# stephane-caron/qpmpc

Hardware: AMD Instinct MI355X
Metric: MPC QP builds+solves/sec (batched) (higher is better)
Workload: dtype f64

## Files before the change

qpmpc_amd/csrc/mpcqp_quad.hip:

```cpp
#include <hip/hip_runtime.h>
#include <math.h>
#include <stdint.h>
#include <type_traits>

#include "mpcqp.h"
#include "mpcqp_internal.h"
#include "mpcqp_quad_common.h"

namespace mpcqp {

namespace quad {

constexpr int MMAX = 32;
constexpr int MK = 2;

}

using namespace quad;

template <int NX, bool ORD, int WPB, bool SLIM, bool MODEL = false, bool GEN = false>
__global__ void __launch_bounds__(64 * WPB, SLIM ? 2 : 1)
    mpcqp_quad_kernel(const double *__restrict__ gA, const double *__restrict__ gB, const double *__restrict__ gC,
                      const double *__restrict__ ge, const double *__restrict__ gx0, const double *__restrict__ ggoal,
                      const double *__restrict__ gtgt, double *__restrict__ oU, double *__restrict__ olam, int32_t *__restrict__ ostatus,
                      int32_t *__restrict__ oiters, const KernelArgs ka, const int64_t batch)
{
    using T = double;
    extern __shared__ __attribute__((aligned(16))) unsigned char smem_raw[];
    {
        const int64_t b0 = ka.A.batch_stride, b1 = ka.B.batch_stride, b2 = ka.C.batch_stride, b3 = ka.e.batch_stride,
                      b4 = ka.x0.batch_stride, b5 = ka.goal.batch_stride;
        const int64_t s0 = ka.A.step_stride, s1 = ka.B.step_stride, s2 = ka.C.step_stride, s3 = ka.e.step_stride;
        asm volatile("" ::"s"(b0), "s"(b1), "s"(b2), "s"(b3), "s"(b4), "s"(b5), "s"(s0), "s"(s1), "s"(s2), "s"(s3), "s"(ka.N), "s"(ka.nu),
                     "s"(ka.flags), "s"(ka.probe), "s"(gA), "s"(gB), "s"(gC), "s"(ge), "s"(gx0), "s"(ggoal), "s"(ka.n), "s"(ka.m),
                     "s"(batch));
    }
    const int lane = threadIdx.x & 63;
    const int wv = threadIdx.x >> 6;
    const int rb = lane & 48;
    const int l = lane & 15;
    int64_t prob = 4 * ((int64_t)blockIdx.x * WPB + wv) + (rb >> 4);
    const bool valid = prob < batch;
    prob = valid ? prob : batch - 1;
    if constexpr (ORD) {
        const int64_t o = ka.order[prob];
        prob = o < 0 ? 0 : (o >= batch ? batch - 1 : o);
    }
    using CV = Carve<SLIM>;
    constexpr int LDM = CV::LDM, PER = CV::PER;
    T *sm = (T *)smem_raw + (4 * wv + (rb >> 4)) * PER;
    const int n = ka.n, m = ka.m;
    const int row0 = l, row1 = l + NV;
    const bool isc0 = row0 < m, isc1 = row1 < m;
    const T INF = HUGE_VAL;
    constexpr int GS = 33;
    T *Gimg = sm + CV::OFF_M, *Ml = sm + CV::OFF_M;
    T *LTp = sm + CV::OFF_LT + (l * (31 - l)) / 2 - (l + 1);
    T *LTimg = sm + CV::OFF_LT, *Timg = sm + CV::OFF_T, *kAv = sm + CV::OFF_KA;
    int *actv = reinterpret_cast<int *>(sm + CV::OFF_ACT);

    long long *stamp = ka.probe ? (long long *)ka.probe + prob * 16 : nullptr;
    auto tick = [&](int slot) {
        if (stamp && l == 0 && valid) {
            stamp[slot] = (long long)__builtin_readcyclecounter();
            if (slot == 0 || slot == 6) stamp[slot ? 13 : 12] = (long long)__builtin_amdgcn_s_memrealtime();
        }
    };
    tick(0);

    T hval0, hval1;
    bool notpd = false;
    T RM0[NV], RM1[NV], RLt[NV];
    T wv_ = T(0);
    if constexpr (MODEL) {
        const T *model = gA;
        const ModelLayout ml = make_model_layout(ka.nx, ka.N, n, m);
        const int nxr = ka.nx, nT = ka.N * ka.nx;
        const T *x0 = gx0 + prob * ka.x0.batch_stride;
        const T *goal = ggoal ? ggoal + prob * ka.goal.batch_stride : nullptr;
        const T *tgt = gtgt ? gtgt + prob * ka.targets.batch_stride : nullptr;
        notpd = model[ml.total] != T(0);
        {
            T r0[NV], r1[NV];
            ld16(r0, model + ml.off_M + (size_t)(isc0 ? row0 : 0) * NV);
            ld16(r1, model + ml.off_M + (size_t)(isc1 ? row1 : 0) * NV);
            ld16(RLt, model + ml.off_LinvT + (size_t)l * NV);
#pragma unroll
            for (int k = 0; k < NV; ++k) {
                RM0[k] = isc0 ? r0[k] : T(0);
                RM1[k] = isc1 ? r1[k] : T(0);
            }
        }
        auto bound = [&](int row, bool isc) {
            if (!isc) return INF;
            const int mkr = ka.mk, kq = mkr == 2 ? row >> 1 : row / mkr;
            T hh = ge ? ge[prob * ka.e.batch_stride + kq * ka.e.step_stride + (row - kq * mkr)] : model[ml.off_e + row];
            for (int c = 0; c < nxr; ++c) hh -= model[ml.off_Hx + (size_t)row * nxr + c] * x0[c];
            return hh;
        };
        hval0 = bound(row0, isc0);
        hval1 = bound(row1, isc1);
        for (int c = 0; c < nxr; ++c) wv_ += model[ml.off_Wx + (size_t)l * nxr + c] * x0[c];
        if ((ka.flags & MPCQP_Q_TERMINAL) && goal)
            for (int c = 0; c < nxr; ++c) wv_ -= model[ml.off_Wg + (size_t)l * nxr + c] * goal[c];
        if ((ka.flags & MPCQP_Q_STAGE) && tgt)
            for (int j2 = 0; j2 < nT; ++j2) wv_ -= model[ml.off_Wt + (size_t)l * nT + j2] * tgt[j2];
        tick(1);
    } else {
    T Pr[NV];
    T qa;
    T g15a = T(0), g15b = T(0);
    {
        constexpr bool WIDE = GEN && NX > 6;
        const int nx = WIDE ? ka.nx : NX;
        const int nu = ka.nu, N = ka.N;
        constexpr int MKG = GEN ? 4 : MK;
        const int mk = GEN ? ka.mk : MK;
        auto stepof = [&](int row) { return mk == 2 ? row >> 1 : (mk == 1 ? row : (mk == 4 ? row >> 2 : row / 3)); };
        const T *A = gA + prob * ka.A.batch_stride;
        const T *B = gB + prob * ka.B.batch_stride;
        const bool hasC = !GEN || gC != nullptr;
        const T *Cm = hasC ? gC + prob * ka.C.batch_stride : A;
        const T *x0 = gx0 + prob * ka.x0.batch_stride;
        const T *goal = ggoal ? ggoal + prob * ka.goal.batch_stride : nullptr;
        const int sA = ka.A.step_stride ? nx * nx : 0, sB = ka.B.step_stride ? nx * nu : 0, sC = (hasC && ka.C.step_stride) ? mk * nx : 0;
        const bool termP = ka.flags & MPCQP_P_TERMINAL, termQ = (ka.flags & MPCQP_Q_TERMINAL) && goal;
        const T *Dm = (GEN && ka.D.ptr) ? (const T *)ka.D.ptr + prob * ka.D.batch_stride : nullptr;
        const T *tgt = (GEN && gtgt) ? gtgt + prob * ka.targets.batch_stride : nullptr;
        const int sD = (GEN && ka.D.step_stride) ? mk * nu : 0;
        const bool stageP = GEN && (ka.flags & MPCQP_P_STAGE), stageQ = GEN && (ka.flags & MPCQP_Q_STAGE) && tgt;
        constexpr int NAe = NX * NX, NEe = NAe + MKG * NX;
        const int NEr = hasC ? NAe + mk * NX : NAe;
        const bool col = (l < n);
        const int j = col ? (nu == 1 ? l : l / nu) : -1, ii = col ? l - j * nu : 0;
        const int64_t eb = prob * ka.e.batch_stride;
        const int kq0 = stepof(row0), kq1 = stepof(row1);
        const T eval0 = isc0 ? ge[eb + kq0 * ka.e.step_stride + (row0 - kq0 * mk)] : INF;
        const T eval1 = isc1 ? ge[eb + kq1 * ka.e.step_stride + (row1 - kq1 * mk)] : INF;
        const bool xl15 = (l == NV - 1);
        T v[NX], gref[NX], bcol[NX];
#pragma unroll
        for (int s = 0; s < NX; ++s) {
            v[s] = (xl15 && s < nx) ? x0[s < nx ? s : 0] : T(0);
            gref[s] = (termQ && s < nx) ? goal[s < nx ? s : 0] : T(0);
        }
#pragma unroll
        for (int r = 0; r < NX; ++r) bcol[r] = (col && r < nx) ? B[j * sB + (r < nx ? r : 0) * nu + ii] : T(0);
        T dcol[MKG], d15a = T(0), d15b = T(0), tg[NX];
#pragma unroll
        for (int u = 0; u < NX; ++u) tg[u] = T(0);
#pragma unroll
        for (int i2 = 0; i2 < MKG; ++i2) dcol[i2] = T(0);
        if constexpr (GEN) {
            if (Dm) {
#pragma unroll
                for (int i2 = 0; i2 < MKG; ++i2) dcol[i2] = (col && !xl15 && i2 < mk) ? Dm[j * sD + i2 * nu + ii] : T(0);
                if (n == NV) {
                    const int j15 = nu == 1 ? NV - 1 : (NV - 1) / nu, i15 = NV - 1 - j15 * nu;
                    d15a = (isc0 && kq0 == j15) ? Dm[j15 * sD + (row0 - kq0 * mk) * nu + i15] : T(0);
                    d15b = (isc1 && kq1 == j15) ? Dm[j15 * sD + (row1 - kq1 * mk) * nu + i15] : T(0);
                }
            }
            if (stageQ && !WIDE) {
#pragma unroll
                for (int u = 0; u < NX; ++u) tg[u] = (l + 16 * u < N * NX) ? tgt[l + 16 * u] : T(0);
            }
        }
        if constexpr (!WIDE) {
        constexpr int NOP = (NEe + 15) / 16;
        T op[NOP][NV];
        static_for<0, NOP>([&](auto rc) {
            constexpr int r = decltype(rc)::value;
            const int e = l + 16 * r;
            const bool ok = e < NEr;
            const T *p = (e < NAe) ? A + e : Cm + (ok ? e - NAe : 0);
            const int st = (e < NAe) ? sA : sC;
#pragma unroll
            for (int k = 0; k < NV; ++k) {
                const int kc = (k < N) ? k : N - 1;
                op[r][k] = p[kc * st];
            }
        });
        tick(8);
        const T wu = (T)ka.wu;
        qa = T(0);
#pragma unroll
        for (int b = 0; b < NV; ++b) Pr[b] = (l == b) ? (col ? wu : T(1)) : T(0);
        tick(9);
        auto mac = [&](auto idx, auto kc_, T &acc, T xx) {
            constexpr int IDX = decltype(idx)::value, K = decltype(kc_)::value;
            fmac_bcast<IDX % 16>(acc, op[IDX / 16][K], xx);
        };
        static_for<0, NV>([&](auto kk) {
            constexpr int k = decltype(kk)::value;
            if (k < N) {
                if constexpr (!GEN) {
                    T g[MK];
                    static_for<0, MK>([&](auto i2c) {
                        constexpr int i2 = decltype(i2c)::value;
                        T acc = T(0);
                        static_for<0, NX>([&](auto sc) {
                            constexpr int s2 = decltype(sc)::value;
                            mac(ic<NAe + i2 * NX + s2>{}, kk, acc, v[s2]);
                        });
                        g[i2] = acc;
                    });
#pragma unroll
                    for (int i2 = 0; i2 < MK; ++i2) Gimg[l * GS + k * MK + i2] = g[i2];
                } else {
                    static_for<0, MKG>([&](auto i2c) {
                        constexpr int i2 = decltype(i2c)::value;
                        if (i2 < mk) {
                            T acc = T(0);
                            if (hasC) {
                                static_for<0, NX>([&](auto sc) {
                                    constexpr int s2 = decltype(sc)::value;
                                    mac(ic<NAe + i2 * NX + s2>{}, kk, acc, v[s2]);
                                });
                            }
                            acc += (j == k) ? dcol[i2] : T(0);
                            Gimg[l * GS + k * mk + i2] = acc;
                        }
                    });
                }
                if constexpr (GEN && k >= 1) {
                    if (stageP || stageQ) {
                        const T wxs = (T)ka.wx;
                        static_for<0, NX>([&](auto sc) {
                            constexpr int s2 = decltype(sc)::value;
                            constexpr int te = k * NX + s2;
                            T src = xl15 ? T(0) : v[s2];
                            const T t = wxs * src;
                            if (stageQ) qa += t * (row_bcast<NV - 1>(v[s2]) - row_bcast<te % 16>(tg[te / 16]));
                            if (stageP) {
                                dpp_ready(src);
                                static_for<0, NV>([&](auto bc) { fmac_bcast<decltype(bc)::value>(Pr[decltype(bc)::value], src, t); });
                            }
                        });
                    }
                }
                const T hk = (j == k && !xl15) ? T(1) : T(0);
                T w[NX];
                static_for<0, NX>([&](auto rc) {
                    constexpr int r = decltype(rc)::value;
                    T acc = hk * bcol[r];
                    static_for<0, NX>([&](auto sc) {
                        constexpr int s2 = decltype(sc)::value;
                        mac(ic<r * NX + s2>{}, kk, acc, v[s2]);
                    });
                    w[r] = acc;
                });
#pragma unroll
                for (int r = 0; r < NX; ++r) v[r] = w[r];
            }
        });
        } else {
        tick(8);
        const T wu = (T)ka.wu;
        qa = T(0);
#pragma unroll
        for (int b = 0; b < NV; ++b) Pr[b] = (l == b) ? (col ? wu : T(1)) : T(0);
        tick(9);
        constexpr int NAw = NX * NX, NCw = 4 * NX, NEw = NAw + NCw + NX, NOPW = (NEw + 15) / 16;
        T opw[2][NOPW];
        auto fetch = [&](auto dc, int k) {
            constexpr int d = decltype(dc)::value;
            const int kc = k < N ? k : N - 1;
            static_for<0, NOPW>([&](auto rc) {
                constexpr int r = decltype(rc)::value;
                constexpr int e0 = 16 * r;
                const int e = e0 + l;
                T val;
                if constexpr (e0 < NAw) {
                    const int rr = e / NX, ss = e - rr * NX;
                    const bool ok = rr < nx && ss < nx;
                    val = A[kc * sA + (ok ? rr * nx + ss : 0)];
                    val = ok ? val : T(0);
                } else if constexpr (e0 < NAw + NCw) {
                    const int e2 = e - NAw, i2 = e2 / NX, ss = e2 - i2 * NX;
                    const bool ok = hasC && i2 < mk && ss < nx;
                    val = Cm[ok ? kc * sC + i2 * nx + ss : 0];
                    val = ok ? val : T(0);
                } else {
                    const int ss = e - NAw - NCw;
                    const bool ok = stageQ && ss < nx;
                    val = ok ? tgt[kc * nx + ss] : T(0);
                }
                opw[d][r] = val;
            });
        };
        fetch(ic<0>{}, 0);
        fetch(ic<1>{}, 1);
        const T wxs = (T)ka.wx;
        auto cstep = [&](auto dc, int k) {
            constexpr int d = decltype(dc)::value;
            static_for<0, NOPW>([&](auto rc) { dpp_ready(opw[d][decltype(rc)::value]); });
            static_for<0, 4>([&](auto i2c) {
                constexpr int i2 = decltype(i2c)::value;
                if (i2 < mk) {
                    T acc = T(0);
                    if (hasC) {
                        static_for<0, NX>([&](auto sc) {
                            constexpr int s2 = decltype(sc)::value, E = NAw + i2 * NX + s2;
                            fmac_bcast<E % 16>(acc, opw[d][E / 16], v[s2]);
                        });
                    }
                    acc += (j == k) ? dcol[i2] : T(0);
                    Gimg[l * GS + k * mk + i2] = acc;
                }
            });
            if (k >= 1 && (stageP || stageQ)) {
                static_for<0, NX>([&](auto sc) {
                    constexpr int s2 = decltype(sc)::value, E = NAw + NCw + s2;
                    T src = xl15 ? T(0) : v[s2];
                    const T t = wxs * src;
                    if (stageQ) qa += t * (row_bcast<NV - 1>(v[s2]) - row_bcast<E % 16>(opw[d][E / 16]));
                    if (stageP) {
                        dpp_ready(src);
                        static_for<0, NV>([&](auto bc) { fmac_bcast<decltype(bc)::value>(Pr[decltype(bc)::value], src, t); });
                    }
                });
            }
            const T hk = (j == k && !xl15) ? T(1) : T(0);
            T w[NX];
            static_for<0, NX>([&](auto rc) {
                constexpr int r = decltype(rc)::value;
                T acc = hk * bcol[r];
                static_for<0, NX>([&](auto sc) {
                    constexpr int s2 = decltype(sc)::value, E = r * NX + s2;
                    fmac_bcast<E % 16>(acc, opw[d][E / 16], v[s2]);
                });
                w[r] = acc;
            });
#pragma unroll
            for (int r = 0; r < NX; ++r) v[r] = w[r];
            fetch(dc, k + 2);
        };
        for (int k = 0; k < N; k += 2) {
            cstep(ic<0>{}, k);
            if (k + 1 < N) cstep(ic<1>{}, k + 1);
        }
        }
        tick(10);
        const T wt = (T)ka.wt;
        T x[NX];
#pragma unroll
        for (int s = 0; s < NX; ++s) {
            x[s] = row_bcast<NV - 1>(v[s]);
            v[s] = xl15 ? bcol[s] : v[s];
        }
#pragma unroll
        for (int s = 0; s < NX; ++s) {
            const T t = wt * v[s];
            if (termQ) qa += t * (x[s] - gref[s]);
            if (termP) {
                T src = v[s];
                dpp_ready(src);
                static_for<0, NV>([&](auto bc) { fmac_bcast<decltype(bc)::value>(Pr[decltype(bc)::value], src, t); });
            }
        }
        qa = col ? qa : T(0);
        tick(11);
        wave_sync();
        hval0 = isc0 ? eval0 - Gimg[(NV - 1) * GS + row0] : INF;
        hval1 = isc1 ? eval1 - Gimg[(NV - 1) * GS + row1] : INF;
        if constexpr (GEN) {
            g15a = d15a;
            g15b = d15b;
        }
    }
    tick(1);
    {
#pragma unroll
        for (int k = 0; k < NV; ++k) {
            RM0[k] = (isc0 && k < NV - 1) ? Gimg[k * GS + row0] : (GEN && k == NV - 1 ? g15a : T(0));
            RM1[k] = (isc1 && k < NV - 1) ? Gimg[k * GS + row1] : (GEN && k == NV - 1 ? g15b : T(0));
            RLt[k] = (l == k) ? T(1) : T(0);
        }
        static_for<0, NV>([&](auto jc) {
            constexpr int j = decltype(jc)::value;
            const T pij = Pr[j];
            const T piv = row_bcast<j>(pij);
            if (!(piv > T(0))) notpd = true;
            const T rinv = fast_rsqrt(piv);
            const T nt2 = -(pij * rinv * rinv);
            T nl = -(pij * rinv);
            RM0[j] *= rinv;
            RM1[j] *= rinv;
            RLt[j] *= rinv;
            const T wj = qa * rinv;
            wv_ = (l == j) ? wj : wv_;
            {
                T src = pij, wsrc = wj;
                asm volatile("s_nop 1" : "+v"(src), "+v"(nl), "+v"(wsrc) : "v"(RM0[j]), "v"(RM1[j]), "v"(RLt[j]));
                fmac_bcast<j>(qa, wsrc, nl);
                static_for<j + 1, NV>([&](auto kc) {
                    constexpr int k = decltype(kc)::value;
                    fmac_bcast<k>(Pr[k], src, nt2);
                    fmac_bcast<k>(RM0[k], nl, RM0[j]);
                    fmac_bcast<k>(RM1[k], nl, RM1[j]);
                    fmac_bcast<k>(RLt[k], nl, RLt[j]);
                });
            }
        });
        wave_sync();
    }
    }
    tick(2);
    tick(3);
    int status = MPCQP_MAX_ITER, iters = 0;
    T xsol = T(0);
    bool done = notpd;
    bool finished = notpd;
    if (notpd) status = MPCQP_NOT_PD;

    if (isc0) st16(Ml + row0 * LDM, RM0);
    if (isc1) st16(Ml + row1 * LDM, RM1);
    T ltd = T(0);
    if constexpr (SLIM) {
        static_for<0, NV>([&](auto kc) {
            constexpr int k = decltype(kc)::value;
            ltd = (l == k) ? RLt[k] : ltd;
            if (k > l) LTp[k] = RLt[k];
        });
    } else {
        st16(LTimg + l * NV, RLt);
    }
    const T y0 = -wv_;
    T s0, s1, invn0, invn1;
    {
        const T d0 = dot_bcast(wv_, RM0, hval0), d1 = dot_bcast(wv_, RM1, hval1);
        s0 = isc0 ? d0 : INF;
        s1 = isc1 ? d1 : INF;
        const T nn0 = dot16(RM0, RM0), nn1 = dot16(RM1, RM1);
        invn0 = (nn0 > T(0)) ? fast_rsqrt(nn0) : T(1);
        invn1 = (nn1 > T(0)) ? fast_rsqrt(nn1) : T(1);
    }
    const bool sel0 = isc0 && (hval0 < T(1e29)), sel1 = isc1 && (hval1 < T(1e29));
    const T tol = (T)ka.tol;
    const T tolh0 = tol + tol * fabs(hval0), tolh1 = tol + tol * fabs(hval1);
    const int max_iter = ka.max_iter;
    T RT[NV], RH[NV];
#pragma unroll
    for (int k = 0; k < NV; ++k) {
        RT[k] = T(0);
        RH[k] = (l == k) ? T(1) : T(0);
    }
    T lam = T(0);
    int myact = 0;
    bool occ = false;
    bool e0 = sel0, e1 = sel1;
    int nq = 0, p = 0, ldrop = 0;
    unsigned mask = 0;
    bool needp = true, dropping = false;
    T up = T(0);
    int fails = 0;
    T mp[NV];
    auto select = [&]() {
        const bool want = needp & !done & !dropping;
        const unsigned h0 = ~(unsigned)__double2hiint(s0 * invn0), h1 = ~(unsigned)__double2hiint(s1 * invn1);
        const bool v0 = want & e0 & (s0 < -tolh0), v1 = want & e1 & (s1 < -tolh1);
        const unsigned k0 = v0 ? ((h0 & ~31u) | (unsigned)row0) : 0xffffffffu;
        const unsigned k1 = v1 ? ((h1 & ~31u) | (unsigned)row1) : 0xffffffffu;
        const unsigned mkey = row_min(min(k0, k1));
        const bool none = want & (mkey == 0xffffffffu);
        const bool got = want & !none;
        done = done | none;
        status = none ? (int)MPCQP_SOLVED : status;
        p = got ? (int)(mkey & 31u) : p;
        up = got ? T(0) : up;
        needp = needp & !got;
    };
    auto update = [&](auto bc, auto ec, T zn, T cT, T cH) {
        static_for<decltype(bc)::value, decltype(ec)::value>([&](auto kc) {
            constexpr int k = decltype(kc)::value;
            fmac_bcast<k>(RT[k], zn, cT);
            fmac_bcast<k>(RH[k], zn, cH);
        });
    };
#ifndef QUAD_USPLIT
#define QUAD_USPLIT 8
#endif
    constexpr int USPLIT = QUAD_USPLIT;
    T zn = T(0), cT = T(0), cH = T(0);
    wave_sync();
    tick(4);
    for (;;) {
        for (;;) {
            dpp_ready(zn);
            update(ic<0>{}, ic<USPLIT>{}, zn, cT, cH);
            select();
            ld16(mp, Ml + p * LDM);
            update(ic<USPLIT>{}, ic<NV>{}, zn, cT, cH);
            cT = cH = T(0);
            if (__ballot(!done) == 0ull) break;
            const bool st = !done & !dropping;
            const bool drp = !done & dropping;
            const bool phi = p >= NV;
            const int pl = p & 15;
            const T hd = dot16(RH, mp);
            const T kd0 = dot_bcast(hd, RM0, T(0)), kd1 = dot_bcast(hd, RM1, T(0));
            T inv, t2;
            {
                const T kp = phi ? kd1 : kd0, sq = phi ? s1 : s0, iq = phi ? invn1 : invn0;
                const bool okf = kp * iq * iq > T(DEP_FAST);
                const T iv = fast_rcp(kp);
                inv = row_get(okf ? iv : T(-1), rb, pl);
                t2 = row_get(-sq * iv, rb, pl);
            }
            T rd = dot16(RT, mp);
            pin(rd);
            if (__ballot(st & !(inv > T(0))) != 0ull) {
                T z2 = hd * hd;
                z2 += dpp_mov<ROR8>(z2);
                z2 += dpp_mov<ROR4>(z2);
                z2 += dpp_mov<ROR2>(z2);
                z2 += dpp_mov<ROR1>(z2);
                z2 = row_bcast<0>(z2);
                const T sq = row_get(phi ? s1 : s0, rb, pl), iq = row_get(phi ? invn1 : invn0, rb, pl);
                const bool ok2 = (z2 * iq * iq > T(DEP)) & (z2 > T(0));
                const T iv2 = fast_rcp(z2);
                const bool nearp = !(inv > T(0));
                t2 = nearp ? -sq * iv2 : t2;
                inv = nearp ? (ok2 ? iv2 : T(0)) : inv;
            }
            const bool can_move = (nq < n) & (inv > T(0));
            inv = (can_move & st) ? inv : T(0);
            t2 = can_move ? t2 : INF;
            const int sl = (int)__builtin_ctz(~mask);
            const T r = (occ & st) ? rd : T(0);
            const bool blk = (r > T(0)) & (lam < t2 * r);
            if (__ballot(drp | (st & (!can_move | (iters >= max_iter) | blk))) == 0ull) {
                const T tt = st ? t2 : T(0);
                const bool isnew = st & (l == sl), isp = st & (l == pl);
                iters += st ? 1 : 0;
                zn = hd;
                cT = (l == sl) ? inv : -(r * inv);
                cH = -(hd * inv);
                s0 = fma(tt, kd0, s0);
                s1 = fma(tt, kd1, s1);
                T ln = fma(-tt, r, lam);
                ln = (occ & (ln < T(0))) ? T(0) : ln;
                lam = isnew ? up + tt : ln;
                myact = isnew ? p : myact;
                occ = occ | isnew;
                e0 = e0 & !(isp & !phi);
                e1 = e1 & !(isp & phi);
                mask |= st ? (1u << sl) : 0u;
                nq += st ? 1 : 0;
                needp = needp | st;
                continue;
            }
            bool stepping = st;
            {
                const bool lim = stepping & (iters >= max_iter);
                done = done | lim;
                finished = finished | lim;
                status = lim ? (int)MPCQP_MAX_ITER : status;
                stepping = stepping & !lim;
            }
            iters += stepping ? 1 : 0;
            const bool cand = occ & stepping & (r > T(0));
            T t1 = INF;
            int lq = 0;
            const unsigned long long bl = __ballot(stepping & blk);
            if (bl != 0ull) {
                const T ratio = cand ? lam * fast_rcp(r) : INF;
                unsigned hi, lo;
                ordered(ratio, hi, lo);
                hi = cand ? hi : 0xffffffffu;
                const unsigned mhi = row_min(hi);
                const unsigned k2 = (cand && hi == mhi) ? ((lo & ~31u) | (unsigned)l) : 0xffffffffu;
                const unsigned ml = row_min(k2);
                lq = (int)(ml & 15u);
                const T tl1 = row_get(ratio, rb, lq);
                const bool blocked = ((unsigned)(bl >> rb) & 0xffffu) != 0u;
                t1 = (blocked && mhi != 0xffffffffu) ? tl1 : INF;
            }
            T t = t1 < t2 ? t1 : t2;
            {
                const bool inf = stepping & !(t < INF);
                done = done | inf;
                finished = finished | inf;
                status = inf ? (int)MPCQP_INFEASIBLE : status;
                stepping = stepping & !inf;
            }
            t = stepping ? t : T(0);
            const bool full = stepping & (t2 <= t1);
            zn = hd;
            cT = full ? ((l == sl) ? inv : -(r * inv)) : T(0);
            cH = full ? -(hd * inv) : T(0);
            if (__ballot(drp) != 0ull) {
                T vv[NV];
                T vl = T(0);
                if constexpr (SLIM) {
#pragma unroll
                    for (int k = 0; k < NV; ++k) {
                        vv[k] = row_get(RT[k], rb, ldrop);
                        vl = (l == k) ? vv[k] : vl;
                    }
                } else {
                    ld16(vv, kAv);
                    vl = kAv[l];
                }
                const T tl = dot16(RT, vv);
                const T tld = row_get(tl, rb, ldrop);
                const T itl = fast_rcp(tld);
                if (drp) {
                    zn = vl;
                    cT = (l == ldrop) ? T(-1) : (occ ? -tl * itl : T(0));
                    cH = vl * itl;
                    if (l == ldrop) {
                        lam = T(0);
                        occ = false;
                    }
                    mask &= ~(1u << ldrop);
                    --nq;
                    dropping = false;
                }
            }
            if (stepping) {
                s0 = fma(t, kd0, s0);
                s1 = fma(t, kd1, s1);
                lam -= t * r;
                lam = (occ && lam < T(0)) ? T(0) : lam;
                up += t;
            }
            if (full) {
                if (l == sl) {
                    lam = up;
                    myact = p;
                    occ = true;
                }
                if (l == pl) {
                    e0 = e0 & phi;
                    e1 = e1 & !phi;
                }
                mask |= 1u << sl;
                ++nq;
                needp = true;
            }
            const bool partial = stepping & !full;
            if (__ballot(partial) != 0ull) {
                const int cl = row_get(myact, rb, lq);
                if constexpr (!SLIM) {
                    wave_sync();
                    if (partial && l == lq) st16(kAv, RT);
                }
                if (partial) {
                    if (l == (cl & 15)) {
                        e0 = (cl < NV) ? sel0 : e0;
                        e1 = (cl < NV) ? e1 : sel1;
                    }
                    dropping = true;
                    ldrop = lq;
                }
                if constexpr (!SLIM) wave_sync();
            }
        }
        tick(5);
        if (__ballot(!finished) == 0ull) break;
        int aa[NV];
        if constexpr (SLIM) {
            const int mine = occ ? myact : 0;
            static_for<0, NV>([&](auto ac) { aa[decltype(ac)::value] = __builtin_amdgcn_update_dpp(0, mine, 0x150 + decltype(ac)::value, 0xf, 0xf, false); });
        } else {
            actv[l] = occ ? myact : 0;
            wave_sync();
            const int4 *ap = reinterpret_cast<const int4 *>(actv);
#pragma unroll
            for (int q = 0; q < NV / 4; ++q) {
                const int4 t4 = ap[q];
                aa[4 * q] = t4.x;
                aa[4 * q + 1] = t4.y;
                aa[4 * q + 2] = t4.z;
                aa[4 * q + 3] = t4.w;
            }
        }
        auto ma_dot = [&](T cf) {
            T ma[NV];
#pragma unroll
            for (int a = 0; a < NV; ++a) ma[a] = Ml[aa[a] * LDM + l];
            return dot_bcast(cf, ma, T(0));
        };
        T fresh0, fresh1;
        auto slacks = [&](T yv) {
            const T f0 = dot_bcast(yv, RM0, T(0)), f1 = dot_bcast(yv, RM1, T(0));
            fresh0 = isc0 ? hval0 - f0 : INF;
            fresh1 = isc1 ? hval1 - f1 : INF;
        };
        auto of_act = [&](T x0v, T x1v) {
            const T a = row_get(x0v, rb, myact & 15), b = row_get(x1v, rb, myact & 15);
            return (myact < NV) ? a : b;
        };
        T y = y0 - ma_dot(occ ? lam : T(0));
        slacks(y);
        T rho = of_act(fresh0, fresh1);
        rho = occ ? rho : T(0);
        constexpr double REFTOL = 1e-11;
        const T hact = of_act(hval0, hval1);
        const bool needref = occ & !finished & !(fabs(rho) <= T(REFTOL) * (T(1) + fabs(hact)));
        const unsigned long long nr = __ballot(needref);
        if (nr != 0ull) {
            rho = (((unsigned)(nr >> rb) & 0xffffu) != 0u) ? rho : T(0);
            T uk = T(0);
            if constexpr (SLIM) {
                static_for<0, NV>([&](auto kc) {
                    constexpr int k = decltype(kc)::value;
                    T v = RT[k] * rho;
                    v += dpp_mov<ROR8>(v);
                    v += dpp_mov<ROR4>(v);
                    v += dpp_mov<ROR2>(v);
                    v += dpp_mov<ROR1>(v);
                    uk = (l == k) ? v : uk;
                });
            } else {
                st16(Timg + l * NV, RT);
                wave_sync();
                T tc[NV];
#pragma unroll
                for (int a = 0; a < NV; ++a) tc[a] = Timg[a * NV + l];
                uk = dot_bcast(rho, tc, T(0));
            }
            T dl = -dot_bcast(uk, RT, T(0));
            dl = occ ? dl : T(0);
            if (!finished) {
                const T lraw = lam + dl;
                lam = (occ && lraw < T(0)) ? T(0) : lraw;
            }
            y += uk;
            wave_sync();
            slacks(y);
        }
        bool dirty = row_any((e0 && !(fresh0 >= -T(4) * tolh0)) || (e1 && !(fresh1 >= -T(4) * tolh1)), rb);
        {
            const T ra = of_act(fresh0, fresh1);
            const T ta = of_act(tolh0, tolh1);
            const bool off = row_any(occ && !(fabs(ra) <= T(1e3) * ta), rb);
            const bool neg = row_any(occ && !(lam >= T(0)), rb);
            if (stamp && l == 0 && valid && !finished && done) {
                T worst = T(0);
                stamp[14] = (long long)(dirty ? 1 : 0) | (off ? 2 : 0) | (neg ? 4 : 0) | ((long long)fails << 8) | ((long long)nq << 16);
                (void)worst;
            }
            dirty = dirty || off || neg;
        }
        auto primal = [&]() {
            T lt[NV];
            if constexpr (SLIM) {
                static_for<0, NV>([&](auto kc) {
                    constexpr int k = decltype(kc)::value;
                    lt[k] = (k > l) ? LTp[k > l ? k : l + 1] : ((k == l) ? ltd : T(0));
                });
            } else {
                ld16(lt, LTimg + l * NV);
            }
            return dot_bcast(y, lt, T(0));
        };
        if (!finished && done) {
            if (!dirty) {
                xsol = primal();
                status = MPCQP_SOLVED;
                finished = true;
            } else if (++fails < 4) {
                s0 = fresh0;
                s1 = fresh1;
                status = MPCQP_MAX_ITER;
                done = false;
                needp = true;
            } else {
                xsol = primal();
                status = MPCQP_MAX_ITER;
                finished = true;
            }
        }
        wave_sync();
        if (__ballot(!finished) == 0ull) break;
    }
    tick(6);
    const bool ok = (status == MPCQP_SOLVED);
    T lo0 = T(0), lo1 = T(0);
    if (olam) {
        T *lamv = Ml;
        lamv[row0] = T(0);
        lamv[row1] = T(0);
        wave_sync();
        if (occ) lamv[myact] = lam;
        wave_sync();
        lo0 = ok ? lamv[row0] : T(0);
        lo1 = ok ? lamv[row1] : T(0);
    }
    if (valid) {
        if (l < n) oU[prob * (int64_t)n + l] = ok ? xsol : T(0);
        if (olam) {
            if (isc0) olam[prob * (int64_t)m + row0] = lo0;
            if (isc1) olam[prob * (int64_t)m + row1] = lo1;
        }
        if (l == 0) {
            if (ostatus) ostatus[prob] = status;
            if (oiters) oiters[prob] = iters;
        }
    }
}

[[maybe_unused]] static bool quad_pays(int64_t batch) { return batch > 2 * (int64_t)device_simds_now(); }

static bool quad_general(const KernelArgs &ka)
{
    return ka.nx > 4 || ka.mk != MK || !ka.C.ptr || ka.D.ptr || (ka.flags & (MPCQP_P_STAGE | MPCQP_Q_STAGE));
}

#ifndef MPCQP_QUAD_WIDE_UNIT
bool quad_applies(const KernelArgs &ka)
{
    if (ka.n > NV || ka.m > MMAX || ka.m < 1 || ka.nx < 2 || ka.nx > 16) return false;
    if (ka.mk < 1 || ka.mk > 4 || (!ka.C.ptr && !ka.D.ptr)) return false;
    if (ka.N * ka.mk != ka.m || ka.N > NV) return false;
    if (ka.warm_state || (ka.opt_flags & MPCQP_OPT_SEED_VIOLATED)) return false;
    if (quad_general(ka) && ka.order) return false;
    return true;
}

bool quad_eligible(const KernelArgs &ka, int64_t batch)
{
    if (!quad_applies(ka) || (ka.opt_flags & MPCQP_OPT_TWO_PER_WAVE)) return false;
    return (ka.opt_flags & MPCQP_OPT_FOUR_PER_WAVE) || quad_general(ka) || quad_pays(batch);
}

#endif

template <int NX> static int launch_quad_t(const KernelArgs &ka, int64_t batch, hipStream_t st)
{
    const int64_t waves = (batch + 3) / 4;
    auto go = [&](auto kern, size_t per) {
        const size_t bytes = per * 4 * sizeof(double);
        hipLaunchKernelGGL(kern, dim3((unsigned)waves), dim3(64), bytes, st, (const double *)ka.A.ptr, (const double *)ka.B.ptr,
                           (const double *)ka.C.ptr, (const double *)ka.e.ptr, (const double *)ka.x0.ptr,
                           (const double *)ka.goal.ptr, (const double *)nullptr, (double *)ka.U, (double *)ka.lam, ka.status, ka.iters,
                           ka, batch);
    };
    const bool slim = waves > device_simds_now();
    if (NX > 4 || quad_general(ka)) {
        auto gen = [&](auto kern, size_t per) {
            hipLaunchKernelGGL(kern, dim3((unsigned)waves), dim3(64), per * 4 * sizeof(double), st, (const double *)ka.A.ptr,
                               (const double *)ka.B.ptr, (const double *)ka.C.ptr, (const double *)ka.e.ptr, (const double *)ka.x0.ptr,
                               (const double *)ka.goal.ptr, (const double *)ka.targets.ptr, (double *)ka.U, (double *)ka.lam, ka.status,
                               ka.iters, ka, batch);
        };
        if (slim)
            gen(mpcqp_quad_kernel<NX, false, 1, true, false, true>, Carve<true>::PER);
        else
            gen(mpcqp_quad_kernel<NX, false, 1, false, false, true>, Carve<false>::PER);
    } else if constexpr (NX <= 4) {
        if (ka.order) {
            if (slim)
                go(mpcqp_quad_kernel<NX, true, 1, true>, Carve<true>::PER);
            else
                go(mpcqp_quad_kernel<NX, true, 1, false>, Carve<false>::PER);
        } else if (slim) {
            go(mpcqp_quad_kernel<NX, false, 1, true>, Carve<true>::PER);
        } else {
            go(mpcqp_quad_kernel<NX, false, 1, false>, Carve<false>::PER);
        }
    }
    return (int)hipGetLastError();
}

#ifdef MPCQP_QUAD_WIDE_UNIT
int launch_quad_wide(const KernelArgs &ka, int64_t batch, hipStream_t st)
{
    if (ka.nx == 5) return launch_quad_t<5>(ka, batch, st);
    if (ka.nx == 6) return launch_quad_t<6>(ka, batch, st);
    return ka.nx <= 8 ? launch_quad_t<8>(ka, batch, st) : ka.nx <= 12 ? launch_quad_t<12>(ka, batch, st) : launch_quad_t<16>(ka, batch, st);
}
#else
int launch_quad_wide(const KernelArgs &ka, int64_t batch, hipStream_t st);

int launch_quad(const KernelArgs &ka, int64_t batch, hipStream_t st)
{
    switch (ka.nx) {
    case 2: return launch_quad_t<2>(ka, batch, st);
    case 3: return launch_quad_t<3>(ka, batch, st);
    case 4: return launch_quad_t<4>(ka, batch, st);
    default: return launch_quad_wide(ka, batch, st);
    }
}

bool quad_model_eligible(const KernelArgs &ka, int64_t batch)
{
    if (ka.n > NV || ka.m > MMAX || ka.m < 1 || ka.warm_state || (ka.opt_flags & (MPCQP_OPT_TWO_PER_WAVE | MPCQP_OPT_SEED_VIOLATED)))
        return false;
    return (ka.opt_flags & MPCQP_OPT_FOUR_PER_WAVE) || quad_pays(batch);
}

int launch_quad_model(const KernelArgs &ka, int64_t batch, hipStream_t st)
{
    const int64_t waves = (batch + 3) / 4;
    auto go = [&](auto kern, size_t per) {
        const size_t bytes = per * 4 * sizeof(double);
        hipLaunchKernelGGL(kern, dim3((unsigned)waves), dim3(64), bytes, st, (const double *)ka.model, (const double *)nullptr,
                           (const double *)nullptr, (const double *)ka.e.ptr, (const double *)ka.x0.ptr, (const double *)ka.goal.ptr,
                           (const double *)ka.targets.ptr, (double *)ka.U, (double *)ka.lam, ka.status, ka.iters, ka, batch);
    };
    const bool slim = waves > device_simds_now();
    if (ka.order) {
        if (slim)
            go(mpcqp_quad_kernel<3, true, 1, true, true>, Carve<true>::PER);
        else
            go(mpcqp_quad_kernel<3, true, 1, false, true>, Carve<false>::PER);
    } else if (slim) {
        go(mpcqp_quad_kernel<3, false, 1, true, true>, Carve<true>::PER);
    } else {
        go(mpcqp_quad_kernel<3, false, 1, false, true>, Carve<false>::PER);
    }
    return (int)hipGetLastError();
}

#endif

}
```

Measured before the change: 190.1 million.

## Add specialized steady-state add-only loop before the general active-set loop

Inserts a fast-path loop, in an included header, that handles iterations where constraints are only added and never dropped. It keeps per-lane boolean state as wave-wide ballot masks and splits the two kd dot products into independent accumulators for more ILP. When a blocking or drop condition appears it hands state back to the general loop. This aims to cut per-iteration select and drop logic and divergence, at the cost of code size, register pressure and the risk of subtle state-handoff bugs.

New measurement: 205.8 million (median of 6 runs). 1.08x the previous value.

```diff
diff --git a/qpmpc_amd/csrc/mpcqp_quad.hip b/qpmpc_amd/csrc/mpcqp_quad.hip
--- a/qpmpc_amd/csrc/mpcqp_quad.hip
+++ b/qpmpc_amd/csrc/mpcqp_quad.hip
@@ -486,7 +486,8 @@
     wave_sync();
     tick(4);
     for (;;) {
-        for (;;) {
+#include "mpcqp_quad_steady.h"
+        if (general) for (;;) {
             dpp_ready(zn);
             update(ic<0>{}, ic<USPLIT>{}, zn, cT, cH);
             select();
diff --git a/qpmpc_amd/csrc/mpcqp_quad_steady.h b/qpmpc_amd/csrc/mpcqp_quad_steady.h
--- /dev/null
+++ b/qpmpc_amd/csrc/mpcqp_quad_steady.h
@@ -0,0 +1,88 @@
+bool general = true;
+{
+    const int iters_in = iters;
+    auto maskof = [](bool b) { return (unsigned long long)__builtin_amdgcn_ballot_w64(b); };
+    auto lanes = [](unsigned long long m) { return __builtin_amdgcn_inverse_ballot_w64(m); };
+    unsigned long long donem = maskof(done), occm = maskof(occ), e0m = maskof(e0), e1m = maskof(e1);
+    for (;;) {
+        dpp_ready(zn);
+        update(ic<0>{}, ic<USPLIT>{}, zn, cT, cH);
+        {
+            const bool want = !lanes(donem), e0 = lanes(e0m), e1 = lanes(e1m);
+            const unsigned h0 = ~(unsigned)__double2hiint(s0 * invn0), h1 = ~(unsigned)__double2hiint(s1 * invn1);
+            const bool v0 = want & e0 & (s0 < -tolh0), v1 = want & e1 & (s1 < -tolh1);
+            const unsigned k0 = v0 ? ((h0 & ~31u) | (unsigned)row0) : 0xffffffffu;
+            const unsigned k1 = v1 ? ((h1 & ~31u) | (unsigned)row1) : 0xffffffffu;
+            const unsigned mkey = row_min(min(k0, k1));
+            const bool none = want & (mkey == 0xffffffffu);
+            donem |= maskof(none);
+            status = none ? (int)MPCQP_SOLVED : status;
+            p = (want & !none) ? (int)(mkey & 31u) : p;
+        }
+        ld16(mp, Ml + p * LDM);
+        update(ic<USPLIT>{}, ic<NV>{}, zn, cT, cH);
+        const bool st = !lanes(donem), occ = lanes(occm);
+        if (donem == ~0ull) {
+            general = false;
+            break;
+        }
+        const bool phi = p >= NV;
+        const int pl = p & 15;
+        T hd = dot16(RH, mp);
+        T kd0, kd1;
+        {
+            T a0 = T(0), a1 = T(0), b0 = T(0), b1 = T(0);
+            dpp_ready(hd);
+            static_for<0, NV / 2>([&](auto kk) {
+                constexpr int k = 2 * decltype(kk)::value;
+                fmac_bcast<k>(a0, hd, RM0[k]);
+                fmac_bcast<k + 1>(a1, hd, RM0[k + 1]);
+                fmac_bcast<k>(b0, hd, RM1[k]);
+                fmac_bcast<k + 1>(b1, hd, RM1[k + 1]);
+            });
+            kd0 = a0 + a1;
+            kd1 = b0 + b1;
+        }
+        T inv, t2;
+        {
+            const T kp = phi ? kd1 : kd0, sq = phi ? s1 : s0, iq = phi ? invn1 : invn0;
+            const bool okf = kp * iq * iq > T(DEP_FAST);
+            const T iv = fast_rcp(kp);
+            inv = row_get(okf ? iv : T(-1), rb, pl);
+            t2 = row_get(-sq * iv, rb, pl);
+        }
+        T rd = dot16(RT, mp);
+        pin(rd);
+        const bool can_move = (nq < n) & (inv > T(0));
+        const int sl = (int)__builtin_ctz(~mask);
+        const T r = (occ & st) ? rd : T(0);
+        const bool blk = (r > T(0)) & (lam < t2 * r);
+        if (maskof(st & (!can_move | (iters >= max_iter) | blk)) != 0ull) break;
+        inv = st ? inv : T(0);
+        const T tt = st ? t2 : T(0);
+        const bool isnew = st & (l == sl), isp = st & (l == pl);
+        iters += st ? 1 : 0;
+        zn = hd;
+        cT = (l == sl) ? inv : -(r * inv);
+        cH = -(hd * inv);
+        s0 = fma(tt, kd0, s0);
+        s1 = fma(tt, kd1, s1);
+        T ln = fma(-tt, r, lam);
+        ln = (occ & (ln < T(0))) ? T(0) : ln;
+        lam = isnew ? tt : ln;
+        myact = isnew ? p : myact;
+        occm |= maskof(isnew);
+        e0m &= ~maskof(isp & !phi);
+        e1m &= ~maskof(isp & phi);
+        mask |= st ? (1u << sl) : 0u;
+        nq += st ? 1 : 0;
+    }
+    done = lanes(donem);
+    occ = lanes(occm);
+    e0 = lanes(e0m);
+    e1 = lanes(e1m);
+    const bool went = iters != iters_in;
+    up = (went | !done) ? T(0) : up;
+    needp = done ? (needp | went) : false;
+    cT = cH = T(0);
+}
```
